# Shao-Group/aletsch

Hardware: AMD Instinct MI355X
Metric: bundles/sec (higher is better)
Workload: dtype f64

## Files before the change

### aletsch_amd/csrc/decomp_device.h

```cpp
#pragma once
#include "decomp_common.h"
#ifdef ALD_EMU
#include <cstdio>
#include <cstdlib>
namespace ald { inline int32_t *emu_fail_line = nullptr; }
#endif

#ifndef ALD_CLASS_ID
#error "compile with -DALD_CLASS_ID=<0..13> (one translation unit per size class)"
#endif
#if defined(__HIP__) || defined(__clang__)
  #define ALD_UNROLL _Pragma("unroll")
#else
  #define ALD_UNROLL _Pragma("GCC unroll 16")
#endif
#define ALD_CAT2(a, b) a##b
#define ALD_CAT(a, b) ALD_CAT2(a, b)
#ifdef ALD_RAW_VARIANT
#define ALD_CLASS_NS ALD_CAT(ald_r, ALD_CLASS_ID)
#else
#define ALD_CLASS_NS ALD_CAT(ald_c, ALD_CLASS_ID)
#endif

namespace ALD_CLASS_NS {
using namespace ald;
#ifdef ALD_EMU_COUNT
static long g_cnt_router = 0, g_cnt_unsweep = 0, g_cnt_star[34] = {0}, g_cnt_rdeg[34] = {0}, g_cnt_build = 0, g_cnt_pre[3] = {0}, g_cnt_fix[8] = {0}, g_cnt_fix_declined = 0;
struct CntPrinter { ~CntPrinter() { if(g_cnt_unsweep) { fprintf(stderr, "[emu-count] class %d: unsplittable sweeps %ld router runs %ld (of which reach build(): %ld; prepared at level 0/1/2: %ld %ld %ld)\n", ALD_CLASS_ID, g_cnt_unsweep, g_cnt_router, g_cnt_build, g_cnt_pre[0], g_cnt_pre[1], g_cnt_pre[2]);
    fprintf(stderr, "[emu-count]   stars by fan size:"); for(int i = 0; i < 34; i++) if(g_cnt_star[i]) fprintf(stderr, " %d:%ld", i, g_cnt_star[i]); fprintf(stderr, "\n");
    fprintf(stderr, "[emu-count]   stars through the fixed-size form:"); for(int i = 0; i < 8; i++) if(g_cnt_fix[i]) fprintf(stderr, " %d:%ld", i, g_cnt_fix[i]); fprintf(stderr, " declined:%ld\n", g_cnt_fix_declined);
    fprintf(stderr, "[emu-count]   router runs by degree:"); for(int i = 0; i < 34; i++) if(g_cnt_rdeg[i]) fprintf(stderr, " %d:%ld", i, g_cnt_rdeg[i]); fprintf(stderr, "\n"); } } }; static CntPrinter g_cnt_printer;
#endif

enum { MAXV = ClassDims<ALD_CLASS_ID>::MAXV, MAXE = ClassDims<ALD_CLASS_ID>::MAXE, NW = ClassDims<ALD_CLASS_ID>::NW };
typedef uint16_t IDX;
static constexpr IDX NIL = (IDX)0xFFFF;
#if ALD_CLASS_ID == ALD_HUGE_CLASS
typedef uint32_t EID;
enum { EID_LIMIT = 0x7FFFFFF0 };
#else
typedef uint16_t EID;
enum { EID_LIMIT = 0xFFF0 };
#endif
typedef ColdLayoutT<MAXV, MAXE, NW, 0> CL;
#ifndef ALD_KEEP
  #define ALD_KEEP (ALD_CLASS_ID >= ALD_FIRST_GLOBAL_CLASS ? 1 : 0)
#endif
#ifndef ALD_KEEP_TRIV
  #define ALD_KEEP_TRIV ALD_KEEP
#endif
enum { LP = 16, ARENA_I = 96, ARENA_D = 48, SCR_I = 4 * LP + ARENA_I, SCR_D = 2 * LP + ARENA_D };

struct Hot {
    struct alignas(8) Link { IDX es, et, inx, onx; };
    struct alignas(16) EdgeHot { double w; Link lk; };
    EdgeHot  ed[MAXE];
    EID      eid[MAXE];
    struct alignas(8) VertexHot { IDX in_head, out_head, in_deg, out_deg; };
    VertexHot vx[MAXV];
    uint8_t  nz[MAXV];
    uint8_t  hflag[MAXE];
};
struct HotCtx {
    ALD_GLOBAL uint8_t *cold;
    ALD_GLOBAL const KernelArgs *args;
    double   ro_ratio;
    int32_t  ro_type, ro_degree, ro_npairs, tmp0;
    int32_t  ev_all;
#if ALD_KEEP
    uint32_t ev_dirty[(MAXV + 31) / 32];
  #if ALD_KEEP_TRIV
    int32_t  tv_all; uint32_t tv_dirty[(MAXV + 31) / 32];
  #endif
#endif
    int32_t  g, V0, gstrand;
    int32_t  nv, next_id, slot_hw, free_head, free_cnt, status, any_strand, hs_dirty, n_paths, n_iters, n_trace;
    uint32_t sp_used, hl_used; int32_t hl_n;
    int32_t  s_next;
    double   p_min_w, p_min_cov, p_ratio[8]; int32_t p_max_exons, p_trace_cap;
    int32_t  pw_lds, park_lds;
    int32_t  sinkp, special_linked;
    int32_t  maybe_triv;
    int32_t  maybe_broken;
    double   sw_best_r, sw_hit_r; int32_t sw_best_v, sw_hit, sw_vend, sw_dom_base; uint32_t sw_need_lo, sw_need_hi;
    int32_t  sw_ncand;
    int32_t  scr_i[SCR_I]; double scr_d[SCR_D];
#ifdef ALD_PROF
    unsigned long long prof[32];
#endif
};

#if ALD_CLASS_ID >= ALD_FIRST_GLOBAL_CLASS
#define ALD_MERGED_WALKS 1
#endif
#if defined(ALD_EMU)
static thread_local Hot g_H;
static thread_local HotCtx g_HC;
#define H g_H
#define HC g_HC
#elif ALD_CLASS_ID >= ALD_FIRST_GLOBAL_CLASS
__shared__ ALD_GLOBAL Hot *g_Hp;
__shared__ HotCtx g_HC;
#define H (*g_Hp)
#define HC g_HC
#define ALD_HOT_IN_SLAB 1
#else
__shared__ Hot g_H;
__shared__ HotCtx g_HC;
#define H g_H
#define HC g_HC
#endif

struct ColdVertex { double vw; int32_t lpos, rpos, vtype, v2v, memo, pad_; };
struct alignas(64) ColdEdge {
    double   med, eabd, econf, s0abd;
    uint64_t mask[NW];
    int32_t  mei, ecount, s0id;
    uint32_t sp_off, sp_len;
    uint8_t  estrand;
};
static_assert(sizeof(ColdVertex) == CL::VX_BYTES && sizeof(ColdEdge) == CL::ED_BYTES, "slab layout out of sync");
struct Cold {
    ALD_GLOBAL ColdVertex *vx;
    ALD_GLOBAL ColdEdge *ed;
    ALD_GLOBAL int32_t *sp_id; ALD_GLOBAL double *sp_abd;
    ALD_GLOBAL int32_t *hl, *hl_off, *hl_len, *hl_capk, *hl_cnt;
    ALD_GLOBAL int32_t *wi; ALD_GLOBAL double *wd;
    ALD_GLOBAL unsigned long long *po;
    static constexpr int32_t po_cap = CL::PO_CAP;
    static constexpr uint32_t sp_cap = CL::SP_CAP, hl_cap = CL::HL_CAP;
    static constexpr int32_t hl_maxlists = CL::HL_MAXLISTS, w_cap = CL::W_CAP;
};
ALD_INL Cold cold_view()
{
    ALD_GLOBAL uint8_t *b = HC.cold; Cold C;
    C.vx = (ALD_GLOBAL ColdVertex*)(b + CL::o_vx); C.ed = (ALD_GLOBAL ColdEdge*)(b + CL::o_ed);
    C.sp_id = (ALD_GLOBAL int32_t*)(b + CL::o_spid); C.sp_abd = (ALD_GLOBAL double*)(b + CL::o_spabd);
    C.hl = (ALD_GLOBAL int32_t*)(b + CL::o_hl); C.hl_off = (ALD_GLOBAL int32_t*)(b + CL::o_hloff); C.hl_len = (ALD_GLOBAL int32_t*)(b + CL::o_hllen);
    C.hl_capk = (ALD_GLOBAL int32_t*)(b + CL::o_hlcapk); C.hl_cnt = (ALD_GLOBAL int32_t*)(b + CL::o_hlcnt);
    C.wi = (ALD_GLOBAL int32_t*)(b + CL::o_wi); C.wd = (ALD_GLOBAL double*)(b + CL::o_wd);
    C.po = (ALD_GLOBAL unsigned long long*)(b + CL::o_po);
    return C;
}
#define COLD const Cold C = cold_view()

#if defined(ALD_PROF) && !defined(ALD_EMU)
  #define PROF_DECL unsigned long long prof_t_ = __builtin_readcyclecounter()
  #define PROF_ADD(k) do { unsigned long long t1_ = __builtin_readcyclecounter(); if(lane_id() == 0) HC.prof[k] += t1_ - prof_t_; prof_t_ = t1_; } while(0)
  #define PROF_RESET() (prof_t_ = __builtin_readcyclecounter())
#else
  #define PROF_DECL do {} while(0)
  #define PROF_ADD(k) do {} while(0)
  #define PROF_RESET() do {} while(0)
#endif
enum { PF_LOAD = 0, PF_BROKEN, PF_TRIV_EVAL, PF_TRIV_MUT, PF_SMALL_EVAL, PF_SMALL_MUT, PF_UNSPLIT, PF_COLLECT0, PF_G_BALANCE, PF_G_DP, PF_G_SPLITMERGE, PF_G_COLLECT, PF_FINISH,
       PF_T_BALANCE, PF_T_PAIRS, PF_T_SETUP, PF_T_MERGE_LOAD, PF_T_MERGE_ADD, PF_T_MERGE_ISECT, PF_T_MERGE_MASK, PF_T_MERGE_SUMS, PF_T_MERGE_KILL, PF_T_HS, PF_T_TAIL,
       PF_S5_DUP, PF_S5_BODY, PF_S5_RELINK, PF_S6_WALK, PF_S6_LINK, PF_S7, PF_SM_KILL, PF_SM_REEVAL, PF_COUNT };

ALD_INL void fail_(int st, int line)
{
#ifdef ALD_EMU
    if(HC.status == 0 && getenv("ALD_EMU_VERBOSE")) fprintf(stderr, "[emu] graph %d: status %d raised at decomp_device.h:%d\n", HC.g, st, line);
    if(HC.status == 0 && ald::emu_fail_line) ald::emu_fail_line[HC.g] = line;
#endif
    if(HC.status == 0) HC.status = st;
}
#define fail(st) fail_((st), __LINE__)
#define ALD_UNLIKELY(x) __builtin_expect(!!(x), 0)
ALD_FN void trace_emit(int code, int a, int b, double v)
{
    int cap = HC.p_trace_cap;
    ALD_GLOBAL const KernelArgs *A = HC.args;
    int k = HC.n_trace++;
    if(k < cap) { int64_t o = (int64_t)HC.g * cap + k; A->out.trace_codes[3 * o] = code; A->out.trace_codes[3 * o + 1] = a; A->out.trace_codes[3 * o + 2] = b; A->out.trace_vals[o] = v; }
}
#ifdef ALD_PROF
ALD_INL bool tracing_u() { return false; }
ALD_INL bool tracing() { return false; }
#else
ALD_INL bool tracing_u() { return uni(HC.p_trace_cap) > 0; }
ALD_INL bool tracing() { return HC.p_trace_cap > 0; }
#endif
ALD_INL void trace(int code, int a, int b, double v) { HC.n_iters++; if(tracing()) trace_emit(code, a, b, v); }
// ... 1400 lines not shown
    return true;
}
template<bool A> ALD_INL bool star_fixed_any(int x, int n)
{
#if ALD_STARFIX_MAX >= 2
    if(n == 2) return uni(star_fixed<A, 2>(x));
#endif
#if ALD_STARFIX_MAX >= 3
    if(n == 3) return uni(star_fixed<A, 3>(x));
#endif
#if ALD_STARFIX_MAX >= 4
    if(n == 4) return uni(star_fixed<A, 4>(x));
#endif
    return false;
}
ALD_INL void decompose_trivial_vertex_wave(int x)
{
    x = uni(x);
    const int nin = uni(H.vx[x].in_deg), nout = uni(H.vx[x].out_deg);
#if ALD_STARFIX_MAX >= 2
    if(nin == 1 && nout >= 2 && nout <= ALD_STARFIX_MAX) { if(star_fixed_any<true>(x, nout)) return; }
    else if(nout == 1 && nin >= 2 && nin <= ALD_STARFIX_MAX) { if(star_fixed_any<false>(x, nin)) return; }
#endif
#ifdef ALD_STAR_SEQ_MAX
    if((nin == 1 && nout >= 1 && nout <= ALD_STAR_SEQ_MAX) || (nout == 1 && nin >= 1 && nin <= ALD_STAR_SEQ_MAX)) { if(lane_id() == 0) decompose_trivial_vertex(x); wsync(); return; }
#endif
#if !defined(ALD_EMU) && !defined(ALD_STAR_SCRATCH_FORM)
    if(nin == 1 && nout >= 1 && nout <= STAR_MAX) star_reg<true>(x);
    else if(nout == 1 && nin >= 1 && nin <= STAR_MAX) star_reg<false>(x);
#else
    if(nin == 1 && nout >= 1 && nout <= STAR_MAX) star_wave_in(x);
    else if(nout == 1 && nin >= 1 && nin <= STAR_MAX) star_wave_out(x);
#endif
    else { if(lane_id() == 0) decompose_trivial_vertex(x); wsync(); }
}

template<bool SMALL> ALD_INL void decompose_vertex_extend_body(int root, int n)
{
    COLD;
    const Pairs P = pairs_at(SMALL, false);
    int32_t *a = P.a, *b = P.b; double *w = P.w;
    const int deg = (int)uni(H.vx[root].in_deg) + (int)uni(H.vx[root].out_deg);
    const Arena AR = arena_at(SMALL);
    if(ALD_UNLIKELY(4 * deg > AR.cap_i || deg > AR.cap_d || deg > C.w_cap / 16)) { fail(ALD_ST_CAPACITY); return; }
    int nloc = 0; int32_t *loc_e = AR.i;
    for(int e = u_first_in(root); e >= 0; e = u_next_in(e)) { loc_e[nloc++] = e; }
    int nin = nloc;
    for(int e = u_first_out(root); e >= 0; e = u_next_out(e)) { loc_e[nloc++] = e; }
    int32_t *mdeg = AR.i + deg;
    int32_t *evx = AR.i + 2 * deg;
    double *mweight = AR.d;
    for(int i = 0; i < nloc; i++) { mdeg[i] = 0; evx[i] = -1; mweight[i] = 0; }
    const double mw = HC.p_min_w;
    double total_weight = 0;
    for(int i = 0; i < n; i++) {
        if(ALD_UNLIKELY(!(w[i] >= mw - kSMIN))) { fail(ALD_ST_INVARIANT + ALD_INV_WEIGHT); return; }
        int u1 = PLOC(a[i]), u2 = PLOC(b[i]);
        total_weight += w[i];
        if(mdeg[u1] == 0) mweight[u1] = w[i]; else mweight[u1] += w[i];
        if(mdeg[u2] == 0) mweight[u2] = w[i]; else mweight[u2] += w[i];
        mdeg[u1]++; mdeg[u2]++;
    }
    int rlen = uni(C.vx[root].rpos) - uni(C.vx[root].lpos);
    double vertex_weight = uni(C.vx[root].vw) * rlen;
    for(int i = 0; i < nloc; i++) mweight[i] = mweight[i] / total_weight * vertex_weight;
    int m = HC.nv, nn = m;
    for(int i = 0; i < nloc; i++) { if(ALD_UNLIKELY(mdeg[i] == 0)) { fail(ALD_ST_INVARIANT + ALD_INV_OTHER); return; } if(mdeg[i] >= 2) evx[i] = nn++; }
    int newedges = 0;
    for(int i = 0; i < n; i++) { int u1 = PLOC(a[i]), u2 = PLOC(b[i]); if(mdeg[u1] == 1 && mdeg[u2] == 1) evx[u1] = nn++; else if(mdeg[u1] >= 2 && mdeg[u2] >= 2) newedges++; }
    if(ALD_UNLIKELY(nn > MAXV || free_slots() < newedges)) { fail(ALD_ST_CAPACITY); return; }
    HC.maybe_broken = 1; HC.maybe_triv = 1; ev_mark_all();
    for(int i = m; i < nn; i++) { H.vx[i].in_head = NIL; H.vx[i].out_head = NIL; H.vx[i].in_deg = 0; H.vx[i].out_deg = 0; H.nz[i] = 1; C.vx[i].vw = 0; C.vx[i].lpos = 0; C.vx[i].rpos = 0; C.vx[i].vtype = -1; C.vx[i].v2v = -1; }
    HC.nv = nn;
    for(int i = 0; i < nin; i++) {
        int k = evx[i]; if(k < 0) continue; int e = loc_e[i];
        int p = uni(C.vx[uni(H.ed[e].lk.es)].rpos);
        move_edge(e, uni(H.ed[e].lk.es), k); C.vx[k].lpos = p; C.vx[k].rpos = p; C.vx[k].vtype = -1; C.vx[k].vw = 0; C.vx[k].v2v = -2;
    }
    for(int i = nin; i < nloc; i++) {
        int k = evx[i]; if(k < 0) continue; int e = loc_e[i];
        int p = uni(C.vx[uni(H.ed[e].lk.et)].lpos);
        move_edge(e, k, uni(H.ed[e].lk.et)); C.vx[k].lpos = p; C.vx[k].rpos = p; C.vx[k].vtype = -1; C.vx[k].vw = 0; C.vx[k].v2v = -2;
    }
    int rv = uni(C.vx[root].v2v);
    for(int i = 0; i < n; i++) {
        int e1 = PSLOT(a[i]), e2 = PSLOT(b[i]); int u1 = PLOC(a[i]), u2 = PLOC(b[i]); double ww = w[i];
        if(mdeg[u1] == 1 && mdeg[u2] >= 2) {
            borrow_edge_strand(C, e1, e2);
            move_edge(e1, uni(H.ed[e1].lk.es), evx[u2]);
            if(rv >= 0) C.ed[e1].mask[(rv >> 6)] |= (1ull << (rv & 63));
            C.ed[e1].med += mweight[u1]; C.ed[e1].mei += rlen;
        } else if(mdeg[u2] == 1) {
            if(ALD_UNLIKELY(evx[u1] < 0)) { fail(ALD_ST_INVARIANT + ALD_INV_OTHER); return; }
            borrow_edge_strand(C, e2, e1);
            move_edge(e2, evx[u1], uni(H.ed[e2].lk.et));
            if(rv >= 0) C.ed[e2].mask[(rv >> 6)] |= (1ull << (rv & 63));
            C.ed[e2].med += mweight[u2]; C.ed[e2].mei += rlen;
        } else {
            int z = add_edge(evx[u1], evx[u2]);
            if(z < 0) return;
            H.ed[z].w = ww;
            if(ALD_UNLIKELY(!(C.ed[e1].ecount > 0 && uni(C.ed[e2].ecount) > 0))) { fail(ALD_ST_INVARIANT + ALD_INV_COUNT); return; }
            if(!intersect_samples(e1, e2, z)) return;
            if(ALD_UNLIKELY(C.ed[z].ecount <= 0)) { fail(ALD_ST_INVARIANT + ALD_INV_COUNT); return; }
            C.ed[z].econf = 0; C.ed[z].estrand = 0;
            for(int k = 0; k < NW; k++) C.ed[z].mask[k] = 0;
            if(rv >= 0) C.ed[z].mask[(rv >> 6)] |= (1ull << (rv & 63));
            C.ed[z].med = ww / total_weight * vertex_weight; C.ed[z].mei = rlen;
            borrow_edge_strand(C, z, e1); borrow_edge_strand(C, z, e2);
            hs_insert_between(e1, e2, z);
            if(HC.status) return;
        }
    }
    if(ALD_UNLIKELY(H.vx[root].in_deg != 0 || uni(H.vx[root].out_deg) != 0)) { fail(ALD_ST_INVARIANT + ALD_INV_DEGREE); return; }
    H.nz[root] = 0;
    double jump = HC.p_ratio[7];
    if(jump > 1.0) {
        int32_t *order = (int32_t*)(C.wi + 3 * (C.w_cap / 8)); int no = 0;
        for(int part = 0; part < 2; part++) {
            int lo = part == 0 ? 0 : nin, hi = part == 0 ? nin : nloc; int first = no;
            for(int i = lo; i < hi; i++) if(evx[i] >= 0) {
                int k = evx[i]; uint32_t id = uni(H.eid[loc_e[i]]); int j = no - 1;
                while(j >= first && uni(H.eid[mdeg[j]]) > id) { order[j + 1] = order[j]; mdeg[j + 1] = mdeg[j]; j--; }
                order[j + 1] = k; mdeg[j + 1] = loc_e[i]; no++;
            }
        }
        for(int q = 0; q < no; q++) { resolve_single_trivial_vertex(order[q], jump); if(HC.status) return; }
    }
}

ALD_FN void decompose_vertex_extend_small(int root, int n) { decompose_vertex_extend_body<true>(uni(root), uni(n)); }
template<bool LDS> ALD_INL void copy_pairs(bool from_parked, bool to_parked, int n)
{
    const Pairs S = pairs_at(LDS, from_parked), D = pairs_at(LDS, to_parked);
    for(int i = 0; i < n; i++) { D.a[i] = S.a[i]; D.b[i] = S.b[i]; D.w[i] = S.w[i]; }
}
ALD_FN void decompose_vertex_extend_any(int root, int n)
{
    root = uni(root); n = uni(n);
    if(uni(HC.pw_lds) != 0) {
        const Pairs S = pairs_at(true, false), D = pairs_at(false, false);
        if(ALD_UNLIKELY(n > D.cap)) { fail(ALD_ST_CAPACITY); return; }
        for(int i = 0; i < n; i++) { D.a[i] = S.a[i]; D.b[i] = S.b[i]; D.w[i] = S.w[i]; }
        HC.pw_lds = 0;
    }
    decompose_vertex_extend_body<false>(root, n);
}
ALD_INL void decompose_vertex_extend(int root, int n)
{
    root = uni(root); n = uni(n);
    const int deg = (int)uni(H.vx[root].in_deg) + (int)uni(H.vx[root].out_deg);
    if(uni(HC.pw_lds) != 0 && 4 * deg <= ARENA_I && deg <= ARENA_D && !(uni(HC.p_ratio[7]) > 1.0)) decompose_vertex_extend_small(root, n);
    else decompose_vertex_extend_any(root, n);
}

ALD_INL int classify_trivial_fastpath(int x, bool fast)
{
    int d1 = H.vx[x].in_deg, d2 = H.vx[x].out_deg;
    if(d1 != 1 && d2 != 1) return -1;
    int e1 = first_in(x), e2 = first_out(x);
    if(d1 == 1) { int s = H.ed[e1].lk.es; if(H.vx[s].out_deg == 1) return 1; if(fast) { if(!(H.hflag[e1] & HF_OCC)) return 1; return -2; } }
    if(d2 == 1) { int t = H.ed[e2].lk.et; if(H.vx[t].in_deg == 1) return 1; if(fast) { if(!(H.hflag[e2] & HF_OCC)) return 1; return -2; } }
    return 2;
}
ALD_FN int classify_trivial_vertex(int x, bool fast)
{
    x = uni(x); fast = uni(fast);
    int d1 = uni(H.vx[x].in_deg), d2 = uni(H.vx[x].out_deg);
    if(d1 != 1 && d2 != 1) return -1;
    int e1 = u_first_in(x), e2 = u_first_out(x);
    if(d1 == 1) { int s = uni(H.ed[e1].lk.es); if(H.vx[s].out_deg == 1) return 1; if(fast && hs_dominate(e1, 1)) return 1; }
    if(d2 == 1) { int t = uni(H.ed[e2].lk.et); if(H.vx[t].in_deg == 1) return 1; if(fast && hs_dominate(e2, 2)) return 1; }
    return 2;
}
ALD_INL double compute_balance_ratio(int v, bool &ok)
{
#ifndef ALD_MERGED_WALKS
    double w1 = in_weights(v), w2 = out_weights(v);
#else
    double w1 = 0, w2 = 0;
    {
        int a = first_in(v), b = first_out(v);
        while((a >= 0) | (b >= 0)) {
            const int ea = a >= 0 ? a : 0, eb = b >= 0 ? b : 0;
            const double wa = H.ed[ea].w, wb = H.ed[eb].w; const IDX na = H.ed[ea].lk.inx, nb = H.ed[eb].lk.onx;
            if(a >= 0) { w1 += wa; a = na == NIL ? -1 : (int)na; }
            if(b >= 0) { w2 += wb; b = nb == NIL ? -1 : (int)nb; }
        }
    }
#endif
    ok = (w1 >= kSMIN) && (w2 >= kSMIN);
    if(w1 >= w2) return w1 / w2; else return w2 / w1;
}
ALD_FN bool resolve_single_trivial_vertex(int i, double jump_ratio)
{
    i = uni(i); jump_ratio = uni(jump_ratio);
    if(H.vx[i].in_deg == 0 || H.vx[i].out_deg == 0) return false;
    if(H.vx[i].in_deg >= 2 && H.vx[i].out_deg >= 2) return false;
    if(mixed_strand_vertex(i)) return false;
    if(classify_trivial_vertex(i, false) != 1) return false;
    bool ok; double r = compute_balance_ratio(i, ok);
    if(ALD_UNLIKELY(!ok)) { fail(ALD_ST_INVARIANT + ALD_INV_WEIGHT); return false; }
    if(r >= jump_ratio) return false;
    trace(OP_TRIVIAL_FAST, vlog(i), 0, r);
    decompose_trivial_vertex(i);
    return true;
}
ALD_INL int eval_smallest(int i, double &r)
{
    int hin, hout;
    {
        const Hot::VertexHot vr = H.vx[i];
        const int nzv = H.nz[i] & NZ_MEMBER, d1 = vr.in_deg, d2 = vr.out_deg;
        if((nzv == 0) | (d1 <= 1) | (d2 <= 1)) return -1;
        hin = slot_or_neg(vr.in_head); hout = slot_or_neg(vr.out_head);
    }
    int e1 = -1, e2 = -1; double sum1 = 0, sum2 = 0, min1 = DBL_MAX, min2 = DBL_MAX;
#ifndef ALD_MERGED_WALKS
    for(int e = hin; e >= 0; e = next_in(e)) { double w = H.ed[e].w; sum1 += w; if(w > min1) continue; min1 = w; e1 = e; }
    for(int e = hout; e >= 0; e = next_out(e)) { double w = H.ed[e].w; sum2 += w; if(w > min2) continue; min2 = w; e2 = e; }
#else
    {
        int a = hin, b = hout;
        while((a >= 0) | (b >= 0)) {
            const int ea = a >= 0 ? a : 0, eb = b >= 0 ? b : 0;
            const double wa = H.ed[ea].w, wb = H.ed[eb].w; const IDX na = H.ed[ea].lk.inx, nb = H.ed[eb].lk.onx;
            if(a >= 0) { sum1 += wa; if(!(wa > min1)) { min1 = wa; e1 = a; } a = na == NIL ? -1 : (int)na; }
            if(b >= 0) { sum2 += wb; if(!(wb > min2)) { min2 = wb; e2 = b; } b = nb == NIL ? -1 : (int)nb; }
        }
    }
#endif
    if(e1 < 0 || e2 < 0) return -1;
    if(!(sum1 >= kSMIN) || !(sum2 >= kSMIN)) return -3;
    double r1 = min1 / sum1, r2 = min2 / sum2;
    int e; if(r1 < r2) { r = r1; e = e1; } else { r = r2; e = e2; }
    int s = H.ed[e].lk.es, t = H.ed[e].lk.et;
    uint8_t f = H.hflag[e];
    { const int ods = H.vx[s].out_deg, idt = H.vx[t].in_deg; if((ods <= 1) | (idt <= 1)) return -1; }
    if((f & HF_REXT) && (f & HF_LEXT)) return -1;
    if(t == i && (f & HF_REXT)) return -1;
    if(s == i && (f & HF_LEXT)) return -1;
    if(HC.any_strand) {
        COLD;
        int z = C.ed[e].estrand;
        if(z >= 1) { int vs[6]; strand_degree(i, vs); if(s == i && vs[0] + vs[z] <= 1) return -1; if(t == i && vs[3] + vs[z + 3] <= 1) return -1; }
    }
    return e;
}

ALD_INL bool resolve_broken_vertex()
{
    if(!uni(HC.maybe_broken)) return false;
    const int lane = lane_id();
    int vend = HC.nv; int x = -1;
    for(int base = 0; base < vend && x < 0; base += ALD_WAVE) {
        int i = base + lane;
        const bool inr = (i >= 1) & (i < vend) & (i != HC.sinkp); const int ii = inr ? i : 0;
        const Hot::VertexHot vr = H.vx[ii];
        const int nzv = H.nz[ii] & NZ_MEMBER, d1 = vr.in_deg, d2 = vr.out_deg;
        bool p = inr & (nzv != 0) & !((d1 >= 1) & (d2 >= 1));
        uint64_t m = wballot(p);
        if(m) x = base + ffs64(m);
    }
    if(x < 0) { wsync(); if(lane == 0) HC.maybe_broken = 0; wsync(); return false; }
    if(lane == 0) {
        if(H.vx[x].in_deg + H.vx[x].out_deg == 0) fail(ALD_ST_INVARIANT + ALD_INV_OTHER);
        else {
            HC.maybe_triv = 1;
            trace(OP_BROKEN, vlog(x), H.vx[x].in_deg + H.vx[x].out_deg, 0);
            int guard = MAXE;
            while(first_in(x) >= 0 && guard-- > 0) { int e = first_in(x); kill_edge(e); hs_remove(e); }
            while(first_out(x) >= 0 && guard-- > 0) { int e = first_out(x); kill_edge(e); hs_remove(e); }
            H.nz[x] = 0; ev_mark(x);
        }
    }
    wsync();
    return true;
}

ALD_INL int nth_set_bit(uint64_t m, int r)
{
    int pos = 0;
    ALD_UNROLL for(int w = 32; w >= 1; w >>= 1) {
        const uint64_t low = m & ((1ull << w) - 1ull); const int c = (int)__builtin_popcountll(low);
        if(r >= c) { r -= c; m >>= w; pos += w; } else m = low;
    }
    return pos;
}
ALD_INL int classify_with_ratio(int i, bool inr, double &r, bool &bad)
{
    int cls = -9; r = 0; bad = false;
    const int ii = inr ? i : 0;
    const Hot::VertexHot vr = H.vx[ii];
    const int nzv = H.nz[ii] & NZ_MEMBER, d1 = vr.in_deg, d2 = vr.out_deg; const IDX h1 = vr.in_head, h2 = vr.out_head;
    bool elig = inr & (nzv != 0) & (d1 >= 1) & (d2 >= 1) & !((d1 >= 2) & (d2 >= 2));
    if(HC.any_strand) elig = elig && !mixed_strand_vertex(i);
    const int e1 = (elig & (h1 != NIL)) ? (int)h1 : 0, e2 = (elig & (h2 != NIL)) ? (int)h2 : 0;
    const IDX sv = H.ed[e1].lk.es, tv = H.ed[e2].lk.et; const uint8_t f1 = H.hflag[e1], f2 = H.hflag[e2];
    const int s_ = (elig & (sv != NIL)) ? (int)sv : 0, t_ = (elig & (tv != NIL)) ? (int)tv : 0;
    const int ods = H.vx[s_].out_deg, idt = H.vx[t_].in_deg;
    if(elig) {
        if(d1 == 1 && ods == 1) cls = 1;
        else if(d1 == 1) cls = (f1 & HF_OCC) ? -2 : 1;
        else if(d2 == 1 && idt == 1) cls = 1;
        else if(d2 == 1) cls = (f2 & HF_OCC) ? -2 : 1;
        else cls = 2;
// ... 649 lines not shown
        double sum = 0; bool bad = false;
        for(int t = 0; t < 4; t++) {
            #define R4_SUM(al, ks, kt, uw) if(al) { const int y_ = ((ks) == x) ? (kt) : (((kt) == x) ? (ks) : -1); if(y_ == t) { sum += (uw); if(!(R4_VW(t) >= vx)) bad = true; } }
            R4_SUM(al0, ks0, kt0, uw0) R4_SUM(al1, ks1, kt1, uw1) R4_SUM(al2, ks2, kt2, uw2)
            #undef R4_SUM
        }
        if(ALD_UNLIKELY(bad)) { fail(ALD_ST_INVARIANT + ALD_INV_ROUTER); return 0; }
        for(int t = 0; t < 4; t++) {
            #define R4_SHARE(al, ks, kt, uw) if(al) { const int y_ = ((ks) == x) ? (kt) : (((kt) == x) ? (ks) : -1); if(y_ == t) { \
                const double wgt = vx * (uw) / sum; const int a_ = x < t ? x : t, b_ = x < t ? t : x; \
                pa[np] = PMAKE(R4_U2E(a_), a_); pb[np] = PMAKE(R4_U2E(b_), b_); pwt[np] = wgt; np++; \
                const double vt_ = R4_VW(t) - wgt; R4_SET(v0, v1, v2, v3, t, vt_); } }
            R4_SHARE(al0, ks0, kt0, uw0) R4_SHARE(al1, ks1, kt1, uw1) R4_SHARE(al2, ks2, kt2, uw2)
            #undef R4_SHARE
        }
        R4_SET(v0, v1, v2, v3, x, -1.0);
        R4_CLEAR(x);
    }
    #undef R4_VW
    #undef R4_DEG
    #undef R4_U2E
    #undef R4_CLEAR
    if(ALD_UNLIKELY(live != 0)) { fail(ALD_ST_INVARIANT + ALD_INV_ROUTER); return 0; }
    double weight_remain = 0;
    if(!(v0 <= 0)) weight_remain += v0;
    if(!(v1 <= 0)) weight_remain += v1;
    if(!(v2 <= 0)) weight_remain += v2;
    if(!(v3 <= 0)) weight_remain += v3;
    HC.ro_ratio = weight_remain / weight_sum;
    C.ed[e0].econf = uni(ecf[0]) + uni(share[0]);
    C.ed[e1].econf = uni(ecf[1]) + uni(share[1]);
    if(q == 2) C.ed[e2].econf = uni(ecf[2]) + uni(share[2]);
    if(q == 3) C.ed[e3].econf = uni(ecf[3]) + uni(share[3]);
    sort_pairs(PW, np);
    const double mw = HC.p_min_w;
    for(int i = 0; i < np; i++) if(pwt[i] < mw) pwt[i] = mw;
    HC.ro_npairs = np;
    return 1;
}
#undef R4_GET
#undef R4_SET
ALD_FN bool router_small(int root, int want_type, int max_degree, int pre) { return router_body<true>(uni(root), uni(want_type), uni(max_degree), uni(pre)); }
ALD_FN bool router_large(int root, int want_type, int max_degree) { return router_body<false>(uni(root), uni(want_type), uni(max_degree), 0); }
ALD_FN int router_prepare(int root)
{
    COLD;
    root = uni(root);
    const int lane = lane_id();
    const int nin = uni(H.vx[root].in_deg), nout = uni(H.vx[root].out_deg), n = nin + nout;
    const int route_bound = (uni(HC.hl_n) == 0) ? 0 : nin * nout;
    const bool small = (route_bound + n <= LP) && (5 * n + 3 * (route_bound + n) <= ARENA_I) && (3 * n + route_bound + n <= ARENA_D);
    if(!small) return 0;
    const Arena AR = arena_at(true);
    int32_t *u2e = AR.i, *ncnt = AR.i + 2 * n, *nsid = AR.i + 3 * n, *iso = AR.i + 4 * n; double *nabd = AR.d, *econf = AR.d + 2 * n;
    double *ecf = AR.d + ARENA_D - n;
    bool multi = false;
    for(int l = lane; l < n; l += ALD_WAVE) {
        int e;
        if(l < nin) { e = first_in(root); for(int k = 0; k < l && e >= 0; k++) e = next_in(e); }
        else { e = first_out(root); for(int k = nin; k < l && e >= 0; k++) e = next_out(e); }
        if(e < 0) e = 0;
        const int cnt = (int)C.ed[e].sp_len, ec = C.ed[e].ecount;
        u2e[l] = e; ncnt[l] = cnt; nsid[l] = C.ed[e].s0id; nabd[l] = C.ed[e].s0abd; iso[l] = (ec == 0) ? 2 : 0; ecf[l] = C.ed[e].econf;
        if(ec != 0 && cnt != 1) multi = true;
    }
    wsync();
    if(route_bound != 0 || wballot(multi) != 0) return 1;
    int partner[(LP + ALD_WAVE - 1) / ALD_WAVE]; double mabd[(LP + ALD_WAVE - 1) / ALD_WAVE], share[(LP + ALD_WAVE - 1) / ALD_WAVE];
    { int q = 0; for(int v = lane; v < n; v += ALD_WAVE, q++) {
        int pt = -1; double max_abd = 0.0, sum_abd = 0.0;
        const int lo = v < nin ? nin : 0, hi = v < nin ? n : nin;
        const int sv = nsid[v]; const double av = nabd[v];
        if(iso[v] != 2) for(int r = lo; r < hi; r++) {
            if(iso[r] == 2) continue;
            const double ar = nabd[r];
            const double al = v < nin ? av : ar, arr = v < nin ? ar : av;
            const double c = (nsid[r] == sv) ? (0.0 + (0.99 * ((arr < al) ? arr : al) + 0.01 * ((al < arr) ? arr : al))) : 0.0;
            sum_abd += c; if(c > max_abd) { max_abd = c; pt = r; }
        }
        partner[q] = pt; mabd[q] = max_abd; share[q] = log(max_abd / sum_abd);
    } }
    wsync();
    { int q = 0; for(int v = lane; v < n; v += ALD_WAVE, q++) { ncnt[v] = partner[q]; nabd[v] = mabd[q]; econf[v] = share[q]; } }
    wsync();
    return 2;
}
ALD_INL bool router_run(int root, int want_type, int max_degree, int pre = 0)
{
#ifdef ALD_EMU_COUNT
    g_cnt_router++; { int dg_ = (int)H.vx[root].in_deg + (int)H.vx[root].out_deg; g_cnt_rdeg[dg_ < 33 ? dg_ : 33]++; }
#endif
    root = uni(root);
    const int nin = uni(H.vx[root].in_deg), nout = uni(H.vx[root].out_deg), n = nin + nout;
    const int route_bound = (uni(HC.hl_n) == 0) ? 0 : nin * nout;
    const bool small = (route_bound + n <= LP) && (5 * n + 3 * (route_bound + n) <= ARENA_I) && (3 * n + route_bound + n <= ARENA_D);
#ifndef ALD_NO_ROUTER22
    if(pre == 2 && nin == 2 && nout == 2) { const int r22 = uni(router_22(root, want_type, max_degree)); if(r22 >= 0) return r22 != 0; }
#endif
    return small ? uni(router_small(root, want_type, max_degree, pre)) : uni(router_large(root, want_type, max_degree));
}
ALD_FN void save_pairs(int n)
{
    n = uni(n);
    const bool lds = uni(HC.pw_lds) != 0;
    if(ALD_UNLIKELY(n > (lds ? (int)LP : (int)PW_CAP))) { fail(ALD_ST_CAPACITY); return; }
    if(lds) copy_pairs<true>(false, true, n); else copy_pairs<false>(false, true, n);
    HC.park_lds = lds ? 1 : 0;
}
ALD_FN void restore_pairs(int n)
{
    n = uni(n);
    const bool lds = uni(HC.park_lds) != 0;
    HC.pw_lds = lds ? 1 : 0;
    if(lds) copy_pairs<true>(true, false, n); else copy_pairs<false>(true, false, n);
}
ALD_INL void memo_clear()
{
    const int nv = uni(HC.nv);
    for(int i = lane_id(); i < nv; i += ALD_WAVE) H.nz[i] &= NZ_MEMBER;
    wsync();
}
#ifdef ALD_UNSPLIT_CALL
ALD_FN bool sweep_unsplittable(int type, int degree, double max_ratio)
#else
ALD_INL bool sweep_unsplittable(int type, int degree, double max_ratio)
#endif
{
#ifdef ALD_EMU_COUNT
    g_cnt_unsweep++;
#endif
    type = uni(type); degree = uni(degree); max_ratio = uni(max_ratio);
    COLD;
    const int lane = lane_id();
    int vend = HC.nv;
    bool flag = false;
    int root = -1; double ratio = max_ratio; int best_np = 0;
    int cur = 1;
    while(cur < vend) {
        int i = -1;
        for(int base = (cur / ALD_WAVE) * ALD_WAVE; base < vend && i < 0; base += ALD_WAVE) {
            int i0 = base + lane;
            const bool inr = (i0 >= cur) & (i0 < vend); const int ii = inr ? i0 : 0;
            const Hot::VertexHot vr = H.vx[ii];
            const int nzv = H.nz[ii] & NZ_MEMBER, d1 = vr.in_deg, d2 = vr.out_deg;
            uint64_t m = wballot(inr & (nzv != 0) & (d1 >= 2) & (d2 >= 2));
            if(m) i = base + ffs64(m);
        }
        if(i < 0) break;
        int act = 0;
        int pre = 0;
        { const int mm = uni(H.nz[i]);
          const bool skip = (mm & NZ_MEMO_VALID) && (((mm >> NZ_MEMO_TYPE_SHIFT) & 7) != type || ((mm & NZ_MEMO_DEG_GT1) && degree <= 1));
          if(!skip) pre = router_prepare(i); }
        if(lane == 0) {
            PROF_DECL;
            const int mm = uni(H.nz[i]);
            bool rok;
            if((mm & NZ_MEMO_VALID) && (((mm >> NZ_MEMO_TYPE_SHIFT) & 7) != type || ((mm & NZ_MEMO_DEG_GT1) && degree <= 1))) rok = false;
            else {
                rok = router_run(i, type, degree, pre);
                if(rok) H.nz[i] = (uint8_t)((mm & NZ_MEMBER) | NZ_MEMO_VALID | ((uni(HC.ro_type) & 7) << NZ_MEMO_TYPE_SHIFT) | (uni(HC.ro_degree) > 1 ? NZ_MEMO_DEG_GT1 : 0));
            }
            PROF_ADD(PF_G_BALANCE);
            if(rok && HC.ro_type == type && HC.ro_degree <= degree) {
                double rr = HC.ro_ratio;
                if(rr < 0.01) {
                    trace(OP_UNSPLIT_NOW, vlog(i), type, rr);
                    decompose_vertex_extend(i, HC.ro_npairs);
                    PROF_ADD(PF_G_DP);
                    act = 1;
                } else if(!(rr > ratio)) {
                    root = i; ratio = rr; best_np = HC.ro_npairs;
                    save_pairs(best_np);
                }
            }
        }
        wsync();
        act = wread(act, 0);
        if(HC.status) return true;
        if(act) { flag = true; memo_clear(); }
        cur = i + 1;
    }
    if(flag) return true;
    root = wread(root, 0);
    if(root < 0) return false;
    if(lane == 0) {
        PROF_DECL;
        restore_pairs(best_np);
        trace(OP_UNSPLIT_BEST, vlog(root), type, ratio);
        decompose_vertex_extend(root, best_np);
        PROF_ADD(PF_G_DP);
    }
    wsync();
    return true;
}

ALD_FN void collect_path(int e)
{
    e = uni(e);
    COLD;
    ALD_GLOBAL const KernelArgs *A = HC.args;
    int n = HC.V0 - 1;
    int cnt = 0, mi = 0, nexw = 0, last_r = INT_MIN; bool empty = false;
    for(int k = 0; k < NW; k++) { uint64_t mk = uni(C.ed[e].mask[k]); while(mk) { int b = ffs64(mk); mk &= mk - 1; int x = k * 64 + b; cnt++; const int l = uni(C.vx[x].lpos), r = uni(C.vx[x].rpos); mi += r - l; if(C.vx[x].vtype == K_EMPTY_VERTEX) empty = true;
        if(l < r) { if(nexw == 0 || last_r != l) nexw += 2; last_r = r; } } }
    if(ALD_UNLIKELY(C.ed[e].mei != mi || cnt == 0)) { fail(ALD_ST_INVARIANT + ALD_INV_OTHER); return; }
    if(C.vx[0].vtype == K_EMPTY_VERTEX || uni(C.vx[n].vtype) == K_EMPTY_VERTEX) empty = true;
    if(!empty) {
        int nvp = cnt + 2;
        if(ALD_UNLIKELY(HC.n_paths >= C.po_cap)) { fail(ALD_ST_CAPACITY); return; }
        unsigned long long words = rec_words((unsigned)nvp, (unsigned)nexw);
        unsigned long long o = atomic_add_u64(A->out.pool_used, words);
        if(ALD_UNLIKELY(o + words > A->out.pool_cap)) { fail(ALD_ST_POOL_FULL); return; }
        C.po[HC.n_paths] = o;
        ALD_GLOBAL uint32_t *r = A->out.pool + o;
        int st = '.';
        if(C.ed[e].estrand == 1) st = '+';
        if(C.ed[e].estrand == 2) st = '-';
        if(st == '.') st = HC.gstrand;
        r[ALD_REC_GRAPH] = (uint32_t)HC.g; r[ALD_REC_PATH] = (uint32_t)HC.n_paths; r[ALD_REC_NV] = (uint32_t)nvp; r[ALD_REC_LENGTH] = (uint32_t)mi; r[ALD_REC_COUNT] = (uint32_t)uni(C.ed[e].ecount); r[ALD_REC_STRAND] = (uint32_t)st | ((uint32_t)(A->attempt & 0xFF) << 8);
        ALD_GLOBAL double *d = (ALD_GLOBAL double*)(r + ALD_REC_WEIGHT);
        d[rec_f64_slot(ALD_REC_WEIGHT)] = uni(H.ed[e].w); d[rec_f64_slot(ALD_REC_ABD)] = uni(C.ed[e].eabd); d[rec_f64_slot(ALD_REC_CONF)] = exp(C.ed[e].econf); d[rec_f64_slot(ALD_REC_READS)] = uni(C.ed[e].med);
        ALD_GLOBAL uint32_t *pv = r + ALD_REC_HDR; int w = 0;
        pv[w++] = 0;
        for(int k = 0; k < NW; k++) { uint64_t mk = uni(C.ed[e].mask[k]); while(mk) { int b = ffs64(mk); mk &= mk - 1; pv[w++] = (uint32_t)(k * 64 + b); } }
        pv[w++] = (uint32_t)n;
        r[ALD_REC_NEXW] = (uint32_t)nexw; r[ALD_REC_NEXW + 1] = 0;
        { int q = 0; for(int k = 0; k < NW; k++) { uint64_t mk = uni(C.ed[e].mask[k]); while(mk) { int b = ffs64(mk); mk &= mk - 1; int x = k * 64 + b; const int l = uni(C.vx[x].lpos), rr = uni(C.vx[x].rpos);
            if(l >= rr) continue; if(q > 0 && (int)pv[w + q - 1] == l) pv[w + q - 1] = (uint32_t)rr; else { pv[w + q] = (uint32_t)l; pv[w + q + 1] = (uint32_t)rr; q += 2; } } } w += q; }
        if((ALD_REC_HDR + nvp + nexw) & 1) pv[w] = 0;
        if(tracing()) { int save = HC.n_iters; trace(OP_COLLECT, (int)uni(H.eid[e]), nvp, uni(H.ed[e].w)); HC.n_iters = save; }
        HC.n_paths++;
    }
    H.hflag[e] = 0;
    kill_edge(e);
}
ALD_FN void materialize_special()
{
    if(HC.special_linked) return;
    HC.special_linked = 1;
    const int sinkp = HC.sinkp;
    H.vx[0].out_head = NIL; H.vx[sinkp].in_head = NIL; H.vx[0].out_deg = 0; H.vx[sinkp].in_deg = 0;
    for(int e = 0; e < HC.slot_hw; e++) {
        if(H.ed[e].lk.es == NIL) continue;
        if((int)uni(H.ed[e].lk.es) == 0) link_out(0, e);
        if((int)uni(H.ed[e].lk.et) == sinkp) link_in(sinkp, e);
    }
}
ALD_FN void collect_existing_st_paths()
{
    COLD;
    PROF_DECL;
    const int lane = lane_id();
    const int sink = uni(HC.sinkp), hw = uni(HC.slot_hw);
    ALD_GLOBAL int32_t *lst = C.wi; int n = 0;
    for(int base = 0; base < hw; base += ALD_WAVE) {
        int e = base + lane;
        bool p = e < hw && H.ed[e].lk.es == 0 && (int)H.ed[e].lk.et == sink;
        uint64_t m = wballot(p);
#ifdef ALD_EMU
        if(p) lst[n] = e;
#else
        if(p) lst[n + __builtin_popcountll(m & ((1ull << lane) - 1))] = e;
#endif
        n += __builtin_popcountll(m);
    }
    wsync_mem();
    PROF_ADD(PF_S5_DUP);
    if(n == 0) return;
    if(tracing() || 5 * n > Cold::w_cap || uni(HC.n_paths) + n > Cold::po_cap) {
        if(lane == 0) {
            for(int i = 1; i < n; i++) { int x = lst[i]; uint32_t id = uni(H.eid[x]); int j = i - 1; while(j >= 0 && (uint32_t)uni(H.eid[lst[j]]) > id) { lst[j + 1] = lst[j]; j--; } lst[j + 1] = x; }
            for(int i = 0; i < n && !HC.status; i++) collect_path(lst[i]);
        }
        wsync_mem();
        return;
    }
    ALD_GLOBAL const KernelArgs *A = HC.args;
    ALD_GLOBAL int32_t *ids = C.wi + n, *keep = C.wi + 2 * n;
    ALD_GLOBAL int32_t *nvs = C.wi + 3 * n, *nxs = C.wi + 4 * n;
    const int nlast = HC.V0 - 1;
    const bool ends_empty = C.vx[0].vtype == K_EMPTY_VERTEX || C.vx[nlast].vtype == K_EMPTY_VERTEX;
    for(int j = lane; j < n; j += ALD_WAVE) {
        const int e = lst[j]; int cnt = 0, mi = 0, nexw = 0, last_r = INT_MIN; bool empty = ends_empty;
        for(int k = 0; k < NW; k++) { uint64_t mk = C.ed[e].mask[k]; while(mk) { int b = ffs64(mk); mk &= mk - 1; int x = k * 64 + b; cnt++; const int l = C.vx[x].lpos, rr = C.vx[x].rpos; mi += rr - l; if(C.vx[x].vtype == K_EMPTY_VERTEX) empty = true;
            if(l < rr) { if(nexw == 0 || last_r != l) nexw += 2; last_r = rr; } } }
        ids[j] = (int32_t)H.eid[e]; nvs[j] = cnt; nxs[j] = nexw;
        keep[j] = (C.ed[e].mei != mi || cnt == 0) ? -1 : (empty ? 0 : 1);
    }
    wsync_mem();
    PROF_ADD(PF_S5_BODY);
    bool bad = false, full = false; int kept_total = 0;
    for(int j = lane; j < n; j += ALD_WAVE) {
        const int e = lst[j]; const int32_t id = ids[j]; int rank = 0; bool later_bad = false;
        for(int k = 0; k < n; k++) { const int kk = keep[k]; if(kk < 0) later_bad = true; if(kk == 1 && ids[k] < id) rank++; }
        if(later_bad) bad = true;
        if(keep[j] != 1 || later_bad) continue;
        const int cnt = nvs[j], nexw = nxs[j];
        const int nvp = cnt + 2;
        const unsigned long long words = rec_words((unsigned)nvp, (unsigned)nexw);
        const unsigned long long o = atomic_add_u64(A->out.pool_used, words);
        if(ALD_UNLIKELY(o + words > A->out.pool_cap)) { full = true; continue; }
        C.po[HC.n_paths + rank] = o;
        ALD_GLOBAL uint32_t *r = A->out.pool + o;
        int st = '.';
        if(C.ed[e].estrand == 1) st = '+';
        if(C.ed[e].estrand == 2) st = '-';
        if(st == '.') st = HC.gstrand;
        r[ALD_REC_GRAPH] = (uint32_t)HC.g; r[ALD_REC_PATH] = (uint32_t)(HC.n_paths + rank); r[ALD_REC_NV] = (uint32_t)nvp; r[ALD_REC_LENGTH] = (uint32_t)C.ed[e].mei; r[ALD_REC_COUNT] = (uint32_t)C.ed[e].ecount; r[ALD_REC_STRAND] = (uint32_t)st | ((uint32_t)(A->attempt & 0xFF) << 8);
        ALD_GLOBAL double *d = (ALD_GLOBAL double*)(r + ALD_REC_WEIGHT);
        d[rec_f64_slot(ALD_REC_WEIGHT)] = H.ed[e].w; d[rec_f64_slot(ALD_REC_ABD)] = C.ed[e].eabd; d[rec_f64_slot(ALD_REC_CONF)] = exp(C.ed[e].econf); d[rec_f64_slot(ALD_REC_READS)] = C.ed[e].med;
        ALD_GLOBAL uint32_t *pv = r + ALD_REC_HDR; int w = 0;
        pv[w++] = 0;
        for(int k = 0; k < NW; k++) { uint64_t mk = C.ed[e].mask[k]; while(mk) { int b = ffs64(mk); mk &= mk - 1; pv[w++] = (uint32_t)(k * 64 + b); } }
        pv[w++] = (uint32_t)nlast;
        r[ALD_REC_NEXW] = (uint32_t)nexw; r[ALD_REC_NEXW + 1] = 0;
        { int q = 0; for(int k = 0; k < NW; k++) { uint64_t mk = C.ed[e].mask[k]; while(mk) { int b = ffs64(mk); mk &= mk - 1; int x = k * 64 + b; const int l = C.vx[x].lpos, rr = C.vx[x].rpos;
            if(l >= rr) continue; if(q > 0 && (int)pv[w + q - 1] == l) pv[w + q - 1] = (uint32_t)rr; else { pv[w + q] = (uint32_t)l; pv[w + q + 1] = (uint32_t)rr; q += 2; } } } w += q; }
        if((ALD_REC_HDR + nvp + nexw) & 1) pv[w] = 0;
    }
    const bool any_bad = wballot(bad) != 0, any_full = wballot(full) != 0;
    wsync_mem();
    PROF_ADD(PF_S5_RELINK);
    if(lane == 0) {
        for(int k = 0; k < n; k++) if(keep[k] == 1) kept_total++;
        if(any_bad) fail(ALD_ST_INVARIANT + ALD_INV_OTHER);
        else if(any_full) fail(ALD_ST_POOL_FULL);
        else HC.n_paths += kept_total;
        for(int k = 0; k < n; k++) { const int e = lst[k]; H.hflag[e] = 0; kill_edge_i(e); }
    }
    wsync_mem();
    PROF_ADD(PF_S6_WALK);
}
ALD_FN double compute_maximum_path()
{
    COLD;
    int n = HC.nv;
    ALD_GLOBAL int32_t *vd = C.wi, *q = C.wi + n, *back = C.wi + 2 * n; ALD_GLOBAL double *table = C.wd;
    ALD_GLOBAL int32_t *path = C.wi + Cold::w_cap / 2;
    int qt = 0;
    const int sinkp = HC.sinkp;
    for(int i = 0; i < n; i++) { int d = uni(H.vx[i].in_deg); vd[i] = d; if(d == 0 && i != sinkp) q[qt++] = i; table[i] = -1; back[i] = -1; }
    if(vd[sinkp] == 0) q[qt++] = sinkp;
    int k = 0;
    while(k < qt) { int x = q[k++]; for(int e = u_first_out(x); e >= 0; e = u_next_out(e)) { int t = uni(H.ed[e].lk.et); if(--vd[t] == 0) q[qt++] = t; } }
    HC.tmp0 = 0;
// ... 509 lines not shown
```

Baseline: 2.614 million.

## Add wave-parallel fixed-form extend for degree-2x2 vertices with three pairs

Adds a specialized extend_22 path for vertices with in-degree 2, out-degree 2 and three routing pairs. It splits the vertex into two new vertices plus one new edge, spreading the per-edge updates across lanes and prefetching edge fields through cross-lane reads. Before, this work went through the generic single-lane decompose_vertex_extend. Callers now invoke a wave-level wrapper that falls back to the generic path when the fixed form does not apply, which adds extra syncs and code size and risks divergence from the generic semantics.

Result: faster. 2.744 million (median of 6 runs) (+5.0%).

```diff
diff --git a/aletsch_amd/csrc/decomp_device.h b/aletsch_amd/csrc/decomp_device.h
--- a/aletsch_amd/csrc/decomp_device.h
+++ b/aletsch_amd/csrc/decomp_device.h
@@ -25,10 +25,12 @@
 namespace ALD_CLASS_NS {
 using namespace ald;
 #ifdef ALD_EMU_COUNT
-static long g_cnt_router = 0, g_cnt_unsweep = 0, g_cnt_star[34] = {0}, g_cnt_rdeg[34] = {0}, g_cnt_build = 0, g_cnt_pre[3] = {0}, g_cnt_fix[8] = {0}, g_cnt_fix_declined = 0;
+static long g_cnt_router = 0, g_cnt_unsweep = 0, g_cnt_star[34] = {0}, g_cnt_rdeg[34] = {0}, g_cnt_build = 0, g_cnt_pre[3] = {0}, g_cnt_fix[8] = {0}, g_cnt_fix_declined = 0, g_cnt_x22[3] = {0}, g_cnt_x22s[5] = {0};
 struct CntPrinter { ~CntPrinter() { if(g_cnt_unsweep) { fprintf(stderr, "[emu-count] class %d: unsplittable sweeps %ld router runs %ld (of which reach build(): %ld; prepared at level 0/1/2: %ld %ld %ld)\n", ALD_CLASS_ID, g_cnt_unsweep, g_cnt_router, g_cnt_build, g_cnt_pre[0], g_cnt_pre[1], g_cnt_pre[2]);
     fprintf(stderr, "[emu-count]   stars by fan size:"); for(int i = 0; i < 34; i++) if(g_cnt_star[i]) fprintf(stderr, " %d:%ld", i, g_cnt_star[i]); fprintf(stderr, "\n");
     fprintf(stderr, "[emu-count]   stars through the fixed-size form:"); for(int i = 0; i < 8; i++) if(g_cnt_fix[i]) fprintf(stderr, " %d:%ld", i, g_cnt_fix[i]); fprintf(stderr, " declined:%ld\n", g_cnt_fix_declined);
+    fprintf(stderr, "[emu-count]   extends: %ld through the fixed 2x2 form: %ld declined: %ld\n", g_cnt_x22[2], g_cnt_x22[0], g_cnt_x22[1]);
+    fprintf(stderr, "[emu-count]   fixed 2x2 form: strand to i' from o*: %ld to o' from i*: %ld to z from i*: %ld to z from o*: %ld insert_between acted: %ld\n", g_cnt_x22s[0], g_cnt_x22s[1], g_cnt_x22s[2], g_cnt_x22s[3], g_cnt_x22s[4]);
     fprintf(stderr, "[emu-count]   router runs by degree:"); for(int i = 0; i < 34; i++) if(g_cnt_rdeg[i]) fprintf(stderr, " %d:%ld", i, g_cnt_rdeg[i]); fprintf(stderr, "\n"); } } }; static CntPrinter g_cnt_printer;
 #endif
 
@@ -1735,6 +1737,160 @@
     const int deg = (int)uni(H.vx[root].in_deg) + (int)uni(H.vx[root].out_deg);
     if(uni(HC.pw_lds) != 0 && 4 * deg <= ARENA_I && deg <= ARENA_D && !(uni(HC.p_ratio[7]) > 1.0)) decompose_vertex_extend_small(root, n);
     else decompose_vertex_extend_any(root, n);
+}
+#ifndef ALD_NO_EXTEND22
+ALD_FN bool intersect_would_hold(int e1, int e2)
+{
+    e1 = uni(e1); e2 = uni(e2);
+    COLD;
+    const uint32_t n1 = uni(C.ed[e1].sp_len), n2 = uni(C.ed[e2].sp_len);
+    const int i1 = uni(C.ed[e1].s0id), i2 = uni(C.ed[e2].s0id);
+    if(n1 == 1 && n2 == 1) return i1 == i2;
+    const uint32_t o1 = uni(C.ed[e1].sp_off), o2 = uni(C.ed[e2].sp_off);
+    const uint32_t need = n1 < n2 ? n1 : n2;
+    if(uni(HC.sp_used) + need > C.sp_cap) return false;
+    uint32_t i = 0, j = 0, k = 0;
+    while(i < n1 && j < n2) {
+        int a = n1 == 1 ? i1 : uni(C.sp_id[o1 + i]), b = n2 == 1 ? i2 : uni(C.sp_id[o2 + j]);
+        if(a < b) i++; else if(b < a) j++; else { k++; i++; j++; }
+    }
+    return k > 0;
+}
+ALD_FN bool extend_22(int root)
+{
+    root = uni(root);
+    COLD;
+    const int lane = lane_id();
+    int bad = 0;
+    if(uni(HC.pw_lds) == 0 || uni(HC.p_ratio[7]) > 1.0) bad = 1;
+    const Hot::VertexHot vrx = H.vx[root];
+    int ge[4], gfar[4];
+    {
+        int e = slot_or_neg(vrx.in_head);
+        ALD_UNROLL for(int k = 0; k < 2; k++) {
+            if(e < 0) bad = 1;
+            const int es = e >= 0 ? e : 0; const uint64_t lw = *(const uint64_t*)&H.ed[es].lk;
+            ge[k] = es; gfar[k] = (int)(lw & 0xFFFF); e = lk_next((uint32_t)((lw >> 32) & 0xFFFF));
+        }
+        if(e >= 0) bad = 1;
+        e = slot_or_neg(vrx.out_head);
+        ALD_UNROLL for(int k = 2; k < 4; k++) {
+            if(e < 0) bad = 1;
+            const int es = e >= 0 ? e : 0; const uint64_t lw = *(const uint64_t*)&H.ed[es].lk;
+            ge[k] = es; gfar[k] = (int)((lw >> 16) & 0xFFFF); e = lk_next((uint32_t)(lw >> 48));
+        }
+        if(e >= 0) bad = 1;
+    }
+    const int lt_v = C.vx[root].lpos, rt_v = C.vx[root].rpos, rv_v = C.vx[root].v2v; const double vw_v = C.vx[root].vw;
+#ifndef ALD_EMU
+    double pf_med, pf_abd; int pf_mei, pf_st, pf_cnt, pf_id, pf_pos; uint32_t pf_ns; uint64_t pf_mask0;
+    { const int l4 = lane < 4 ? lane : 0; const int f = pick<4>(ge, l4), fv = pick<4>(gfar, l4);
+      pf_med = C.ed[f].med; pf_abd = C.ed[f].s0abd; pf_mei = C.ed[f].mei; pf_st = C.ed[f].estrand; pf_cnt = C.ed[f].ecount; pf_id = C.ed[f].s0id; pf_ns = C.ed[f].sp_len; pf_mask0 = C.ed[f].mask[0];
+      pf_pos = l4 < 2 ? C.vx[fv].rpos : C.vx[fv].lpos; }
+#endif
+    const Pairs P = pairs_at(true, false);
+    const int a0 = P.a[0], a1 = P.a[1], a2 = P.a[2], b0 = P.b[0], b1 = P.b[1], b2 = P.b[2];
+    const double w0 = P.w[0], w1 = P.w[1], w2 = P.w[2];
+    const int la0 = PLOC(a0), la1 = PLOC(a1), la2 = PLOC(a2), lb0 = PLOC(b0) - 2, lb1 = PLOC(b1) - 2, lb2 = PLOC(b2) - 2;
+    if((unsigned)la0 > 1u || (unsigned)la1 > 1u || (unsigned)la2 > 1u || (unsigned)lb0 > 1u || (unsigned)lb1 > 1u || (unsigned)lb2 > 1u) bad = 1;
+    if(PSLOT(a0) != (la0 ? ge[1] : ge[0]) || PSLOT(a1) != (la1 ? ge[1] : ge[0]) || PSLOT(a2) != (la2 ? ge[1] : ge[0])) bad = 1;
+    if(PSLOT(b0) != (lb0 ? ge[3] : ge[2]) || PSLOT(b1) != (lb1 ? ge[3] : ge[2]) || PSLOT(b2) != (lb2 ? ge[3] : ge[2])) bad = 1;
+    const int c0 = uni((la0 << 1) | lb0), c1 = uni((la1 << 1) | lb1), c2 = uni((la2 << 1) | lb2);
+    if(c0 == c1 || c0 == c2 || c1 == c2) bad = 1;
+    const int cm = (6 - c0 - c1 - c2) & 3;
+    const int ip = cm >> 1, op = 2 + (cm & 1), is = 1 - ip, os = 5 - op;
+    const int cz = (is << 1) | (os - 2), ci = (ip << 1) | (os - 2), co = (is << 1) | (op - 2);
+    const double mw = HC.p_min_w;
+    if(!(w0 >= mw - kSMIN) || !(w1 >= mw - kSMIN) || !(w2 >= mw - kSMIN)) bad = 1;
+    double total_weight = 0; total_weight += w0; total_weight += w1; total_weight += w2;
+    const double wz = c0 == cz ? w0 : (c1 == cz ? w1 : w2), wi = c0 == ci ? w0 : (c1 == ci ? w1 : w2), wo = c0 == co ? w0 : (c1 == co ? w1 : w2);
+    const int m = uni(HC.nv), fh = uni(HC.free_head), hw = uni(HC.slot_hw), id = uni(HC.next_id);
+    if(m + 2 > MAXV || (fh < 0 && hw >= MAXE) || id >= EID_LIMIT) bad = 1;
+    const int z = fh >= 0 ? fh : (hw < MAXE ? hw : 0);
+    const bool dupi = uni(gfar[0] == gfar[1]), dupo = uni(gfar[2] == gfar[3]);
+    const int rlen = uni(rt_v) - uni(lt_v), rv = uni(rv_v);
+    const double vertex_weight = uni(vw_v) * rlen;
+#ifdef ALD_EMU
+    const int e_is = ge[is], e_os = ge[os], e_ip = ge[ip], e_op = ge[op];
+    const int st_is = C.ed[e_is].estrand, st_os = C.ed[e_os].estrand, cnt_is = C.ed[e_is].ecount, cnt_os = C.ed[e_os].ecount, id_is = C.ed[e_is].s0id, id_os = C.ed[e_os].s0id;
+    const uint32_t ns_is = C.ed[e_is].sp_len, ns_os = C.ed[e_os].sp_len; const double abd_is = C.ed[e_is].s0abd, abd_os = C.ed[e_os].s0abd;
+#else
+    const int e_is = uni(pick<4>(ge, is)), e_os = uni(pick<4>(ge, os)), e_ip = uni(pick<4>(ge, ip)), e_op = uni(pick<4>(ge, op));
+    const int st_is = wread(pf_st, is), st_os = wread(pf_st, os), cnt_is = wread(pf_cnt, is), cnt_os = wread(pf_cnt, os), id_is = wread(pf_id, is), id_os = wread(pf_id, os);
+    const uint32_t ns_is = (uint32_t)wread((int)pf_ns, is), ns_os = (uint32_t)wread((int)pf_ns, os); const double abd_is = wread(pf_abd, is), abd_os = wread(pf_abd, os);
+#endif
+    if(!(cnt_is > 0 && cnt_os > 0)) bad = 1;
+    const bool inline_sp = (ns_is == 1 && ns_os == 1);
+    if(inline_sp) { if(id_is != id_os) bad = 1; }
+    else if(!bad && !uni(intersect_would_hold(e_is, e_os))) bad = 1;
+    const bool zfirst = uni(pick<4>(gfar, op) == uni(HC.sinkp));
+#ifdef ALD_EMU_COUNT
+    if(bad) g_cnt_x22[1]++; else { g_cnt_x22[0]++; if(st_os != 0) g_cnt_x22s[0]++; if(st_is != 0) g_cnt_x22s[1]++; if(st_os == 0 && st_is != 0) g_cnt_x22s[2]++; if(st_os != 0 && st_is == 0) g_cnt_x22s[3]++; }
+#endif
+    if(wballot(bad != 0) != 0) return false;
+    for(int j = lane; j < 4; j += ALD_WAVE) {
+        const bool in_side = j < 2, star = (j == is) || (j == os);
+        const int e = pick<4>(ge, j), fv = pick<4>(gfar, j);
+        const int nvx = in_side ? (star ? m : m + 1) : (star ? m + 1 : m);
+#ifdef ALD_EMU
+        const double pf_med = C.ed[e].med; const int pf_mei = C.ed[e].mei, pf_pos = in_side ? C.vx[fv].rpos : C.vx[fv].lpos; const uint64_t pf_mask0 = C.ed[e].mask[0];
+#endif
+        if(star) {
+            C.vx[nvx].lpos = pf_pos; C.vx[nvx].rpos = pf_pos; C.vx[nvx].vtype = -1; C.vx[nvx].vw = 0; C.vx[nvx].v2v = -2;
+        } else {
+            const int sp = in_side ? st_os : st_is;
+            if(sp != 0) C.ed[e].estrand = (uint8_t)sp;
+            if(rv >= 0) { const int k = rv >> 6; C.ed[e].mask[k] = (k == 0 ? pf_mask0 : C.ed[e].mask[k]) | (1ull << (rv & 63)); }
+            const double mweight = (in_side ? wi : wo) / total_weight * vertex_weight;
+            C.ed[e].med = pf_med + mweight; C.ed[e].mei = pf_mei + rlen;
+        }
+        if(in_side) {
+            H.ed[e].lk.inx = star ? NIL : (IDX)z;
+            if(!dupi) { H.ed[e].lk.et = (IDX)nvx; relink_out_lane(fv, e, (uint32_t)nvx); }
+        } else {
+            H.ed[e].lk.onx = (star || zfirst) ? NIL : (IDX)z;
+            if(!dupo) { H.ed[e].lk.es = (IDX)nvx; relink_in_lane(fv, e, (uint32_t)nvx); }
+        }
+    }
+    star_tail_sync();
+    if(lane == 0) {
+        if(dupi) { ALD_UNROLL for(int k = 0; k < 2; k++) { const int nk = (k == is) ? m : m + 1; H.ed[ge[k]].lk.et = (IDX)nk; relink_out(gfar[k], ge[k], (uint32_t)nk); } }
+        if(dupo) { ALD_UNROLL for(int k = 2; k < 4; k++) { const int nk = (k == os) ? m + 1 : m; H.ed[ge[k]].lk.es = (IDX)nk; relink_in(gfar[k], ge[k], (uint32_t)nk); } }
+        if(fh >= 0) { const IDX nx = uni(H.ed[z].lk.onx); HC.free_head = nx == NIL ? -1 : (int)nx; HC.free_cnt = uni(HC.free_cnt) - 1; }
+        else HC.slot_hw = hw + 1;
+        HC.next_id = id + 1;
+        H.ed[z].lk.es = (IDX)m; H.ed[z].lk.et = (IDX)(m + 1); H.ed[z].lk.inx = NIL; H.ed[z].lk.onx = zfirst ? (IDX)e_op : NIL;
+        H.eid[z] = (EID)id; H.hflag[z] = 0; H.ed[z].w = wz;
+        H.vx[m].in_head = (IDX)e_is; H.vx[m].out_head = zfirst ? (IDX)z : (IDX)e_op; H.vx[m].in_deg = 1; H.vx[m].out_deg = 2; H.nz[m] = 1;
+        H.vx[m + 1].in_head = (IDX)e_ip; H.vx[m + 1].out_head = (IDX)e_os; H.vx[m + 1].in_deg = 2; H.vx[m + 1].out_deg = 1; H.nz[m + 1] = 1;
+        HC.nv = m + 2; HC.maybe_broken = 1; HC.maybe_triv = 1; ev_mark_all();
+        if(inline_sp) { const double c = (abd_os < abd_is) ? abd_os : abd_is; C.ed[z].sp_off = 0; C.ed[z].sp_len = 1; C.ed[z].ecount = 1; C.ed[z].eabd = 0.0 + c; C.ed[z].s0id = id_is; C.ed[z].s0abd = c; }
+        else intersect_samples(e_is, e_os, z);
+        C.ed[z].econf = 0; C.ed[z].estrand = (uint8_t)(st_os != 0 ? st_os : st_is);
+        for(int k = 0; k < NW; k++) C.ed[z].mask[k] = (rv >= 0 && (rv >> 6) == k) ? (1ull << (rv & 63)) : 0ull;
+        C.ed[z].med = wz / total_weight * vertex_weight; C.ed[z].mei = rlen;
+#ifdef ALD_EMU_COUNT
+        { const int32_t d0 = HC.hs_dirty; HC.hs_dirty = 0; hs_insert_between(e_is, e_os, z); if(HC.hs_dirty) g_cnt_x22s[4]++; HC.hs_dirty |= d0; }
+#else
+        hs_insert_between(e_is, e_os, z);
+#endif
+        clear_vertex(root);
+    }
+    wsync();
+    return true;
+}
+#endif
+ALD_FN void decompose_vertex_extend_wave(int root, int n)
+{
+    root = uni(root); n = uni(n);
+#ifdef ALD_EMU_COUNT
+    g_cnt_x22[2]++;
+#endif
+#ifndef ALD_NO_EXTEND22
+    if(n == 3 && uni(H.vx[root].in_deg) == 2 && uni(H.vx[root].out_deg) == 2) { if(uni(extend_22(root))) return; }
+#endif
+    if(lane_id() == 0) decompose_vertex_extend(root, n);
+    wsync();
 }
 
 ALD_INL int classify_trivial_fastpath(int x, bool fast)
@@ -2690,8 +2846,9 @@
         { const int mm = uni(H.nz[i]);
           const bool skip = (mm & NZ_MEMO_VALID) && (((mm >> NZ_MEMO_TYPE_SHIFT) & 7) != type || ((mm & NZ_MEMO_DEG_GT1) && degree <= 1));
           if(!skip) pre = router_prepare(i); }
+        PROF_DECL;
         if(lane == 0) {
-            PROF_DECL;
+            PROF_RESET();
             const int mm = uni(H.nz[i]);
             bool rok;
             if((mm & NZ_MEMO_VALID) && (((mm >> NZ_MEMO_TYPE_SHIFT) & 7) != type || ((mm & NZ_MEMO_DEG_GT1) && degree <= 1))) rok = false;
@@ -2704,8 +2861,6 @@
                 double rr = HC.ro_ratio;
                 if(rr < 0.01) {
                     trace(OP_UNSPLIT_NOW, vlog(i), type, rr);
-                    decompose_vertex_extend(i, HC.ro_npairs);
-                    PROF_ADD(PF_G_DP);
                     act = 1;
                 } else if(!(rr > ratio)) {
                     root = i; ratio = rr; best_np = HC.ro_npairs;
@@ -2715,6 +2870,7 @@
         }
         wsync();
         act = wread(act, 0);
+        if(act) { decompose_vertex_extend_wave(i, uni(HC.ro_npairs)); PROF_ADD(PF_G_DP); }
         if(HC.status) return true;
         if(act) { flag = true; memo_clear(); }
         cur = i + 1;
@@ -2722,14 +2878,14 @@
     if(flag) return true;
     root = wread(root, 0);
     if(root < 0) return false;
-    if(lane == 0) {
+    best_np = wread(best_np, 0);
+    {
         PROF_DECL;
-        restore_pairs(best_np);
-        trace(OP_UNSPLIT_BEST, vlog(root), type, ratio);
-        decompose_vertex_extend(root, best_np);
+        if(lane == 0) { restore_pairs(best_np); trace(OP_UNSPLIT_BEST, vlog(root), type, ratio); }
+        wsync();
+        decompose_vertex_extend_wave(root, best_np);
         PROF_ADD(PF_G_DP);
     }
-    wsync();
     return true;
 }
 
```
